# fgvieira/ngsLD

Measured on AMD Instinct MI355X. Metric: SNP-pair EM-LD computations/sec @ n_ind=500, higher is better.
Workload: dtype f64

## Files before the change

### ngsld_amd/csrc/ld_pair_moments.hip

```cpp
#include <algorithm>

#include "ld_dispatch.h"

namespace ngsld {

namespace {
constexpr uint32_t kTR = 128, kTC = 64, kKc = 16;
constexpr uint32_t kSites = kTR + kTC;
constexpr uint32_t kLd = kSites + 16;
typedef double v4d __attribute__((ext_vector_type(4)));
typedef double v2d __attribute__((ext_vector_type(2)));
}

template <bool DOSE>
__global__ __launch_bounds__(512) void pair_ld_moments_kernel(MomentArgs A) {
  __shared__ double sE[kKc * kLd];
  __shared__ double sD[DOSE ? kKc * kLd : 1];
  __shared__ uint64_t s_ioff[kTR];
  __shared__ uint32_t s_end[kTR];
  __shared__ uint32_t s_cmax;
  const uint32_t t = threadIdx.x, lane = t & 63u;
  const uint32_t wave = (uint32_t)__builtin_amdgcn_readfirstlane((int)(t >> 6));
  const uint32_t rb = A.row0 + blockIdx.y * kTR;
  const uint64_t c0 = (uint64_t)rb + 1u + (uint64_t)blockIdx.x * kTC;
  if (t == 0) s_cmax = 0;
  __syncthreads();
  if (t < kTR) {
    const uint32_t row = rb + t;
    const bool in = row < A.row1;
    const uint32_t e = in ? A.row_end[row] : 0u;
    s_end[t] = e;
    s_ioff[t] = in ? A.item_off[row] : 0ull;
    atomicMax(&s_cmax, e);
  }
  __syncthreads();
  const uint32_t cmax = s_cmax;
  if (c0 >= cmax) return;

  const bool loader = t < 2 * kSites;
  const uint32_t sl = t < kSites ? t : (loader ? t - kSites : 0u), half = t < kSites ? 0u : 1u;
  uint64_t site = sl < kTR ? (uint64_t)rb + sl : c0 + (sl - kTR);
  if (site >= A.n_sites) site = A.n_sites - 1;
  const double m = A.maf[site];
  const bool flip = m > 0.5;
  const DoseWeights u = dose_weights(flip ? 1.0 - m : m);
  const double *pl = A.planes + site * A.site_stride + half * 8u;
  const double *p0 = pl + (flip ? 2u * A.np : 0u), *p1 = pl + A.np, *p2 = pl + (flip ? 0u : 2u * A.np);
  v2d q0[4], q1[4], q2[4];
  auto fetch = [&](uint32_t kc) {
#pragma unroll
    for (int i = 0; i < 4; ++i) {
      q0[i] = reinterpret_cast<const v2d *>(p0 + kc * kKc)[i];
      q1[i] = reinterpret_cast<const v2d *>(p1 + kc * kKc)[i];
      q2[i] = reinterpret_cast<const v2d *>(p2 + kc * kKc)[i];
    }
  };
  auto stage = [&](uint32_t kc) {
#pragma unroll
    for (int i = 0; i < 8; ++i) {
      const double a0 = q0[i >> 1][i & 1], a1 = q1[i >> 1][i & 1], a2 = q2[i >> 1][i & 1];
      const uint32_t k = half * 8u + (uint32_t)i;
      sE[k * kLd + sl] = fma(2.0, a2, a1);
      if (DOSE) {
        double den, num;
        dose_terms(u, a0, a1, a2, den, num);
        sD[k * kLd + sl] = kc * kKc + k < A.n_ind ? num / den : 0.0;
      }
    }
  };

  const uint32_t wr = wave & 3u, wc = wave >> 2;
  bool live[2][2];
#pragma unroll
  for (int ri = 0; ri < 2; ++ri)
#pragma unroll
    for (int cj = 0; cj < 2; ++cj) {
      const uint64_t r_lo = (uint64_t)rb + wr * 32u + ri * 16u, c_lo = c0 + wc * 32u + cj * 16u;
      live[ri][cj] = r_lo < A.row1 && c_lo + 15u > r_lo && c_lo < cmax;
    }
  v4d totE[2][2], totD[2][2];
#pragma unroll
  for (int ri = 0; ri < 2; ++ri)
#pragma unroll
    for (int cj = 0; cj < 2; ++cj) totE[ri][cj] = totD[ri][cj] = v4d{0.0, 0.0, 0.0, 0.0};
  const uint32_t oa = (lane >> 4) * kLd + wr * 32u + (lane & 15u);
  const uint32_t ob = (lane >> 4) * kLd + kTR + wc * 32u + (lane & 15u);

  const uint32_t nk = A.np / kKc;
  if (loader) fetch(0);
  for (uint32_t kc = 0; kc < nk; ++kc) {
    lds_barrier();
    if (loader) {
      stage(kc);
      if (kc + 1 < nk) fetch(kc + 1);
    }
    lds_barrier();
    v4d inE[2][2], inD[2][2];
#pragma unroll
    for (int ks = 0; ks < 4; ++ks) {
      double ae[2], be[2], ad[2], bd[2];
#pragma unroll
      for (int x = 0; x < 2; ++x) {
        ae[x] = sE[ks * 4 * kLd + oa + x * 16];
        be[x] = sE[ks * 4 * kLd + ob + x * 16];
        if (DOSE) {
          ad[x] = sD[ks * 4 * kLd + oa + x * 16];
          bd[x] = sD[ks * 4 * kLd + ob + x * 16];
        }
      }
#pragma unroll
      for (int ri = 0; ri < 2; ++ri)
#pragma unroll
        for (int cj = 0; cj < 2; ++cj) {
          if (!live[ri][cj]) continue;
          const v4d z = {0.0, 0.0, 0.0, 0.0};
          inE[ri][cj] = __builtin_amdgcn_mfma_f64_16x16x4f64(ae[ri], be[cj], ks == 0 ? z : inE[ri][cj], 0, 0, 0);
          if (DOSE) inD[ri][cj] = __builtin_amdgcn_mfma_f64_16x16x4f64(ad[ri], bd[cj], ks == 0 ? z : inD[ri][cj], 0, 0, 0);
        }
    }
#pragma unroll
    for (int ri = 0; ri < 2; ++ri)
#pragma unroll
      for (int cj = 0; cj < 2; ++cj) {
        if (!live[ri][cj]) continue;
        totE[ri][cj] += inE[ri][cj];
        if (DOSE) totD[ri][cj] += inD[ri][cj];
      }
  }

#pragma unroll
  for (int ri = 0; ri < 2; ++ri)
#pragma unroll
    for (int cj = 0; cj < 2; ++cj) {
      if (!live[ri][cj]) continue;
#pragma unroll
      for (int r = 0; r < 4; ++r) {
        const uint32_t lr = wr * 32u + ri * 16u + (lane >> 4) + 4u * r;
        const uint64_t s1 = (uint64_t)rb + lr, s2 = c0 + wc * 32u + cj * 16u + (lane & 15u);
        if (s1 >= A.row1 || s2 <= s1 || s2 >= s_end[lr]) continue;
        const uint64_t off = s2 - s1 - 1;
        const Item *it = A.items_all + s_ioff[lr] + (off >> 6);
        const uint64_t mask = it->mask, bit = 1ull << (off & 63u);
        if (!(mask & bit)) continue;
        const uint64_t idx = it->first_record + (uint64_t)__popcll(mask & (bit - 1)) - A.rec0;
        reinterpret_cast<v2d *>(A.out)[idx] = v2d{totE[ri][cj][r], DOSE ? totD[ri][cj][r] : 0.0};
      }
    }
}

hipError_t launch_pair_moments(const MomentArgs &a, const uint32_t *h_row_end, hipStream_t stream) {
  if (a.row1 <= a.row0) return hipSuccess;
  uint64_t most = 0;
  for (uint32_t rb = a.row0; rb < a.row1; rb += kTR) {
    uint32_t end = 0;
    for (uint32_t r = rb; r < a.row1 && r < rb + kTR; ++r) end = std::max(end, h_row_end[r]);
    if (end > rb + 1) most = std::max<uint64_t>(most, ((uint64_t)end - rb - 1 + kTC - 1) / kTC);
  }
  if (most == 0) return hipSuccess;
  if (most > (1ull << 22)) return hipErrorInvalidValue;
  const uint64_t blocks_y = std::min<uint64_t>(65535, std::max<uint64_t>(1, (1ull << 22) / most));
  for (uint64_t r0 = a.row0; r0 < a.row1; r0 += blocks_y * kTR) {
    MomentArgs b = a;
    b.row0 = (uint32_t)r0;
    const uint64_t by = std::min<uint64_t>(blocks_y, ((uint64_t)a.row1 - r0 + kTR - 1) / kTR);
    const dim3 grid((unsigned)most, (unsigned)by), block(512);
    if (a.dose)
      hipLaunchKernelGGL((pair_ld_moments_kernel<true>), grid, block, 0, stream, b);
    else
      hipLaunchKernelGGL((pair_ld_moments_kernel<false>), grid, block, 0, stream, b);
    const hipError_t e = hipGetLastError();
    if (e != hipSuccess) return e;
  }
  return hipSuccess;
}

}
```

Before: 217.3 million.

## Double-buffer LDS tiles and interleave staging with MFMA via sched groups

Splits the shared-memory tiles into two buffers so the next k-chunk is staged while the current chunk's MFMA products run, dropping one barrier per iteration. The loading work is redistributed across all 512 threads (three sites per thread, two k values each), and a rotated row padding is added to avoid LDS bank conflicts. A fully-live fast path removes per-tile predicates and uses sched_group_barrier to interleave MFMA with VALU staging work. In exchange it doubles LDS usage, which may reduce occupancy, and it adds scheduling complexity.

```diff
diff --git a/ngsld_amd/csrc/ld_pair_moments.hip b/ngsld_amd/csrc/ld_pair_moments.hip
--- a/ngsld_amd/csrc/ld_pair_moments.hip
+++ b/ngsld_amd/csrc/ld_pair_moments.hip
@@ -1,4 +1,5 @@
 #include <algorithm>
+#include <type_traits>
 
 #include "ld_dispatch.h"
 
@@ -7,15 +8,17 @@
 namespace {
 constexpr uint32_t kTR = 128, kTC = 64, kKc = 16;
 constexpr uint32_t kSites = kTR + kTC;
-constexpr uint32_t kLd = kSites + 16;
+constexpr uint32_t kRot = 4, kLd = kSites + kRot * (kKc / 2 - 1) + 20;
+static_assert(kLd % 32 == 16, "moments pass: rows k and k + 1 in opposite halves of the LDS banks");
+constexpr uint32_t kBuf = kKc * kLd;
 typedef double v4d __attribute__((ext_vector_type(4)));
 typedef double v2d __attribute__((ext_vector_type(2)));
 }
 
 template <bool DOSE>
 __global__ __launch_bounds__(512) void pair_ld_moments_kernel(MomentArgs A) {
-  __shared__ double sE[kKc * kLd];
-  __shared__ double sD[DOSE ? kKc * kLd : 1];
+  __shared__ double sE[2 * kBuf];
+  __shared__ double sD[DOSE ? 2 * kBuf : 1];
   __shared__ uint64_t s_ioff[kTR];
   __shared__ uint32_t s_end[kTR];
   __shared__ uint32_t s_cmax;
@@ -37,34 +40,49 @@
   const uint32_t cmax = s_cmax;
   if (c0 >= cmax) return;
 
-  const bool loader = t < 2 * kSites;
-  const uint32_t sl = t < kSites ? t : (loader ? t - kSites : 0u), half = t < kSites ? 0u : 1u;
-  uint64_t site = sl < kTR ? (uint64_t)rb + sl : c0 + (sl - kTR);
-  if (site >= A.n_sites) site = A.n_sites - 1;
-  const double m = A.maf[site];
-  const bool flip = m > 0.5;
-  const DoseWeights u = dose_weights(flip ? 1.0 - m : m);
-  const double *pl = A.planes + site * A.site_stride + half * 8u;
-  const double *p0 = pl + (flip ? 2u * A.np : 0u), *p1 = pl + A.np, *p2 = pl + (flip ? 0u : 2u * A.np);
-  v2d q0[4], q1[4], q2[4];
+  const uint32_t k0 = 2u * (lane & 7u), sl0 = 8u * wave + (lane >> 3);
+  const double *pl[3];
+  double mq[3];
+  uint32_t off0[3];
+#pragma unroll
+  for (int s = 0; s < 3; ++s) {
+    uint64_t site = s < 2 ? (uint64_t)rb + 64u * s + sl0 : c0 + sl0;
+    if (site >= A.n_sites) site = A.n_sites - 1;
+    const double m = A.maf[site];
+    const bool flip = m > 0.5;
+    mq[s] = flip ? 1.0 - m : m;
+    pl[s] = A.planes + site * A.site_stride + k0;
+    off0[s] = flip ? 2u * A.np : 0u;
+  }
+  v2d q0[3], q1[3], q2[3];
   auto fetch = [&](uint32_t kc) {
 #pragma unroll
-    for (int i = 0; i < 4; ++i) {
-      q0[i] = reinterpret_cast<const v2d *>(p0 + kc * kKc)[i];
-      q1[i] = reinterpret_cast<const v2d *>(p1 + kc * kKc)[i];
-      q2[i] = reinterpret_cast<const v2d *>(p2 + kc * kKc)[i];
+    for (int s = 0; s < 3; ++s) {
+      uint32_t o = off0[s];
+      asm volatile("" : "+v"(o));
+      const double *p = pl[s] + kc * kKc;
+      q0[s] = *reinterpret_cast<const v2d *>(p + o);
+      q1[s] = *reinterpret_cast<const v2d *>(p + A.np);
+      q2[s] = *reinterpret_cast<const v2d *>(p + (2u * A.np - o));
     }
   };
   auto stage = [&](uint32_t kc) {
-#pragma unroll
-    for (int i = 0; i < 8; ++i) {
-      const double a0 = q0[i >> 1][i & 1], a1 = q1[i >> 1][i & 1], a2 = q2[i >> 1][i & 1];
-      const uint32_t k = half * 8u + (uint32_t)i;
-      sE[k * kLd + sl] = fma(2.0, a2, a1);
-      if (DOSE) {
-        double den, num;
-        dose_terms(u, a0, a1, a2, den, num);
-        sD[k * kLd + sl] = kc * kKc + k < A.n_ind ? num / den : 0.0;
+    double *bE = sE + (kc & 1u) * kBuf, *bD = sD + (DOSE ? (kc & 1u) * kBuf : 0u);
+#pragma unroll
+    for (int s = 0; s < 3; ++s) {
+      double m = mq[s];
+      asm volatile("" : "+v"(m));
+      const DoseWeights u = dose_weights(m);
+#pragma unroll
+      for (int h = 0; h < 2; ++h) {
+        const double a0 = q0[s][h], a1 = q1[s][h], a2 = q2[s][h];
+        const uint32_t k = k0 + (uint32_t)h, at = k * kLd + kRot * (k0 >> 1) + 64u * s + sl0;
+        bE[at] = fma(2.0, a2, a1);
+        if (DOSE) {
+          double den, num;
+          dose_terms(u, a0, a1, a2, den, num);
+          bD[at] = kc * kKc + k < A.n_ind ? num / den : 0.0;
+        }
       }
     }
   };
@@ -78,41 +96,38 @@
       const uint64_t r_lo = (uint64_t)rb + wr * 32u + ri * 16u, c_lo = c0 + wc * 32u + cj * 16u;
       live[ri][cj] = r_lo < A.row1 && c_lo + 15u > r_lo && c_lo < cmax;
     }
+  const bool all_live = live[0][0] && live[0][1] && live[1][0] && live[1][1];
   v4d totE[2][2], totD[2][2];
 #pragma unroll
   for (int ri = 0; ri < 2; ++ri)
 #pragma unroll
     for (int cj = 0; cj < 2; ++cj) totE[ri][cj] = totD[ri][cj] = v4d{0.0, 0.0, 0.0, 0.0};
-  const uint32_t oa = (lane >> 4) * kLd + wr * 32u + (lane & 15u);
-  const uint32_t ob = (lane >> 4) * kLd + kTR + wc * 32u + (lane & 15u);
-
-  const uint32_t nk = A.np / kKc;
-  if (loader) fetch(0);
-  for (uint32_t kc = 0; kc < nk; ++kc) {
-    lds_barrier();
-    if (loader) {
-      stage(kc);
-      if (kc + 1 < nk) fetch(kc + 1);
-    }
-    lds_barrier();
+  const uint32_t ok = (lane >> 4) * kLd + kRot * (lane >> 5);
+  const uint32_t oa = ok + wr * 32u + (lane & 15u);
+  const uint32_t ob = ok + kTR + wc * 32u + (lane & 15u);
+  constexpr uint32_t kStep = 4 * kLd + 2 * kRot;
+
+  auto products = [&](uint32_t kc, auto all) {
+    constexpr bool ALL = decltype(all)::value;
+    const double *bE = sE + (kc & 1u) * kBuf, *bD = sD + (DOSE ? (kc & 1u) * kBuf : 0u);
     v4d inE[2][2], inD[2][2];
 #pragma unroll
     for (int ks = 0; ks < 4; ++ks) {
       double ae[2], be[2], ad[2], bd[2];
 #pragma unroll
       for (int x = 0; x < 2; ++x) {
-        ae[x] = sE[ks * 4 * kLd + oa + x * 16];
-        be[x] = sE[ks * 4 * kLd + ob + x * 16];
+        ae[x] = bE[ks * kStep + oa + x * 16];
+        be[x] = bE[ks * kStep + ob + x * 16];
         if (DOSE) {
-          ad[x] = sD[ks * 4 * kLd + oa + x * 16];
-          bd[x] = sD[ks * 4 * kLd + ob + x * 16];
+          ad[x] = bD[ks * kStep + oa + x * 16];
+          bd[x] = bD[ks * kStep + ob + x * 16];
         }
       }
 #pragma unroll
       for (int ri = 0; ri < 2; ++ri)
 #pragma unroll
         for (int cj = 0; cj < 2; ++cj) {
-          if (!live[ri][cj]) continue;
+          if (!ALL && !live[ri][cj]) continue;
           const v4d z = {0.0, 0.0, 0.0, 0.0};
           inE[ri][cj] = __builtin_amdgcn_mfma_f64_16x16x4f64(ae[ri], be[cj], ks == 0 ? z : inE[ri][cj], 0, 0, 0);
           if (DOSE) inD[ri][cj] = __builtin_amdgcn_mfma_f64_16x16x4f64(ad[ri], bd[cj], ks == 0 ? z : inD[ri][cj], 0, 0, 0);
@@ -122,11 +137,39 @@
     for (int ri = 0; ri < 2; ++ri)
 #pragma unroll
       for (int cj = 0; cj < 2; ++cj) {
-        if (!live[ri][cj]) continue;
+        if (!ALL && !live[ri][cj]) continue;
         totE[ri][cj] += inE[ri][cj];
         if (DOSE) totD[ri][cj] += inD[ri][cj];
       }
-  }
+  };
+
+  constexpr int kMfma = DOSE ? 32 : 16, kValuPer = DOSE ? 5 : 2;
+  const uint32_t nk = A.np / kKc;
+  fetch(0);
+  stage(0);
+  if (nk > 1) fetch(1);
+  lds_barrier();
+  for (uint32_t kc = 0; kc + 1 < nk; ++kc) {
+    if (all_live) {
+      products(kc, std::true_type{});
+      stage(kc + 1);
+      fetch(std::min(kc + 2, nk - 1));
+#pragma unroll
+      for (int i = 0; i < kMfma; ++i) {
+        __builtin_amdgcn_sched_group_barrier(0x008, 1, 0);
+        __builtin_amdgcn_sched_group_barrier(0x002, kValuPer, 0);
+      }
+    } else {
+      products(kc, std::false_type{});
+      stage(kc + 1);
+      fetch(std::min(kc + 2, nk - 1));
+    }
+    lds_barrier();
+  }
+  if (all_live)
+    products(nk - 1, std::true_type{});
+  else
+    products(nk - 1, std::false_type{});
 
 #pragma unroll
   for (int ri = 0; ri < 2; ++ri)
```

Result: no change. 218.3 million (median of 6 runs) (+0.5%).
